# Vidvox/hap

Measured on AMD Instinct MI355X. Metric: RGBA GB/s + frames/sec, 8K Hap Q encode+decode, higher is better.
Workload: dtype u8; 1 GPU; C4: 7680x4320 0x1, 24 chunks, Snappy, 60-frame stream, device-resident; fragment_index=True, parallelism=single GPU

## Files before the change

hap_amd/csrc/bc_encode_core.hpp:

```cpp
#pragma once
#include <hip/hip_runtime.h>
#include <stdint.h>

#include "bc_refine_core.hpp"

namespace hapbc {

constexpr int kFmtDXT1 = 0, kFmtDXT5 = 1, kFmtYCoCg = 2, kFmtRGTC1 = 3;
constexpr int kFmtYCoCgAlpha = 4;

__device__ __forceinline__ int mad24(int a, int b, int c)
{
    int r;
    asm("v_mad_i32_i24 %0, %1, %2, %3" : "=v"(r) : "v"(a), "v"(b), "v"(c));
    return r;
}
template <int K>
__device__ __forceinline__ int mad24k(int a, int c)
{
    int r;
    asm("v_mad_i32_i24 %0, %1, %2, %3" : "=v"(r) : "v"(a), "i"(K), "v"(c));
    return r;
}

__device__ __forceinline__ int quant5(int v) { int t = mad24k<31>(v, 128); return (t + (t >> 8)) >> 8; }
__device__ __forceinline__ int quant6(int v) { int t = mad24k<63>(v, 128); return (t + (t >> 8)) >> 8; }
__device__ __forceinline__ int expand5(int q) { return (q << 3) | (q >> 2); }
__device__ __forceinline__ int expand6(int q) { return (q << 2) | (q >> 4); }

typedef unsigned short pk_u16 __attribute__((ext_vector_type(2)));
typedef short pk_i16 __attribute__((ext_vector_type(2)));

__device__ __forceinline__ pk_u16 pk_shl(pk_u16 v, unsigned sh)
{
    unsigned r;
    asm("v_pk_lshlrev_b16 %0, %1, %2 op_sel_hi:[0,1]" : "=v"(r) : "v"(sh), "v"(__builtin_bit_cast(unsigned, v)));
    return __builtin_bit_cast(pk_u16, r);
}


__device__ __forceinline__ unsigned ramp_codes(unsigned w)
{
    return w ^ (~((w >> 1) | (w >> 2)) & 0x249249u);
}

template <int BIAS = 0>
__device__ __forceinline__ uint2 alpha_block(const int (&a)[16])
{
    int lo = a[0], hi = a[0];
#pragma unroll
    for (int i = 1; i < 16; i++) {
        lo = min(lo, a[i]);
        hi = max(hi, a[i]);
    }
    const int a0 = hi, a1 = lo;
    unsigned lo24 = 0, hi24 = 0;
    if (a0 != a1) {
        const int d = a0 - a1;
        const unsigned m = (unsigned)(524288.0f * __builtin_amdgcn_rcpf((float)d)) + 1u;
        const int neg_m14 = -(int)(14u * m);
        const int start = mad24(a0, (int)(14u * m), (int)__umul24((unsigned)max(d - 6, 0), m)) + (1 << 20);
#pragma unroll
        for (int i = 0; i < 16; i++) {
            const unsigned r1 = (unsigned)mad24(a[i], neg_m14, start) >> 20;
            if (i < 8)
                lo24 = __builtin_amdgcn_alignbit(r1, lo24, 3);
            else
                hi24 = __builtin_amdgcn_alignbit(r1, hi24, 3);
        }
        lo24 = ramp_codes(lo24 >> 8);
        hi24 = ramp_codes(hi24 >> 8);
    }
    const unsigned long long bits = (unsigned long long)lo24 | ((unsigned long long)hi24 << 24);
    const unsigned long long v = (unsigned long long)(unsigned)(a0 + (a1 << 8) + BIAS * 257) | (bits << 16);
    return make_uint2((unsigned)v, (unsigned)(v >> 32));
}

struct projection {
    unsigned adir;
    unsigned flip;
    int start;
    int top;
    unsigned m24;
};

__device__ __forceinline__ unsigned index_scale(unsigned len2)
{
    unsigned m = (unsigned)(50331648.0f * __builtin_amdgcn_rcpf((float)len2));
    const int rem = (int)(50331648u - m * len2);
    m += (rem >= (int)len2 ? 1u : 0u) - (rem < 0 ? 1u : 0u);
    return m;
}

template <int CHANNELS = 3>
__device__ __forceinline__ projection make_projection(unsigned p0, unsigned p1)
{
    projection pr;
    int dir[CHANNELS];
    unsigned adir = 0, flip = 0;
    int neg = 0, base = 0;
#pragma unroll
    for (int c = 0; c < CHANNELS; c++) {
        const int a = (int)((p0 >> (8 * c)) & 255u), b = (int)((p1 >> (8 * c)) & 255u);
        dir[c] = a - b;
        const int ad = abs(dir[c]);
        adir |= (unsigned)ad << (8 * c);
        flip |= (dir[c] < 0 ? 0xFFu : 0u) << (8 * c);
        neg += dir[c] < 0 ? ad : 0;
        base = mad24(b, dir[c], base);
    }
    const unsigned len2 = __builtin_amdgcn_udot4(adir, adir, 0u, false);
    const unsigned sixth = __umulhi(len2, 0xAAAAAAABu) >> 2;
    pr.adir = adir;
    pr.flip = flip;
    pr.start = (int)sixth - base - 255 * neg;
    pr.top = (int)(len2 + sixth);
    pr.m24 = index_scale(len2);
    return pr;
}

#define HAPBC_CLAMPED_DOTS(OP)                                                                                           \
    asm(OP " %0, %4, %8, %9\n\t" OP " %1, %5, %8, %9\n\t" OP " %2, %6, %8, %9\n\t" OP " %3, %7, %8, %9\n\t"              \
        "v_med3_i32 %0, %0, 0, %10\n\tv_med3_i32 %1, %1, 0, %10\n\tv_med3_i32 %2, %2, 0, %10\n\tv_med3_i32 %3, %3, 0, %10" \
        : "=&v"(t[0]), "=&v"(t[1]), "=&v"(t[2]), "=&v"(t[3])                                                             \
        : "v"(q0), "v"(q1), "v"(q2), "v"(q3), "v"(dir), "v"(start), "v"(top))
__device__ __forceinline__ void clamped_dot4(unsigned (&t)[4], unsigned q0, unsigned q1, unsigned q2, unsigned q3, unsigned dir, int start, int top)
{
    HAPBC_CLAMPED_DOTS("v_dot4_u32_u8");
}
__device__ __forceinline__ void clamped_dot2(unsigned (&t)[4], unsigned q0, unsigned q1, unsigned q2, unsigned q3, unsigned dir, int start, int top)
{
    HAPBC_CLAMPED_DOTS("v_dot2_i32_i16");
}
#undef HAPBC_CLAMPED_DOTS

template <typename DOTS>
__device__ __forceinline__ unsigned gather_indices(unsigned m24, DOTS dots)
{
    const unsigned m30 = m24 << 6;
    unsigned pos2 = 0;
#pragma unroll
    for (int g = 3; g >= 0; g--) {
        unsigned t[4];
        dots(t, 4 * g);
#pragma unroll
        for (int k = 3; k >= 0; k--)
            pos2 = __builtin_amdgcn_alignbit(pos2, t[k] * m30, 30);
    }
    const unsigned hi = pos2 & 0xAAAAAAAAu;
    return (hi ^ ((pos2 << 1) & 0xAAAAAAAAu)) | ((~hi >> 1) & 0x55555555u);
}

template <bool FLIPPED = false>
__device__ __forceinline__ unsigned project4(const unsigned (&px)[16], const projection &pr)
{
    return gather_indices(pr.m24, [&](unsigned (&t)[4], int i) {
        clamped_dot4(t, FLIPPED ? px[i] : px[i] ^ pr.flip, FLIPPED ? px[i + 1] : px[i + 1] ^ pr.flip,
                     FLIPPED ? px[i + 2] : px[i + 2] ^ pr.flip, FLIPPED ? px[i + 3] : px[i + 3] ^ pr.flip, pr.adir, pr.start, pr.top);
    });
}

__device__ __forceinline__ unsigned pack3(int a, int b, int c) { return (unsigned)a | ((unsigned)b << 8) | ((unsigned)c << 16); }

__device__ __forceinline__ unsigned expand_565(unsigned c, bool blue)
{
    return pack3(expand5(c >> 11), expand6((c >> 5) & 63), blue ? expand5(c & 31) : 0);
}

template <bool REFINE = false>
__device__ __forceinline__ uint2 colour_block(const unsigned (&px)[16])
{
    int lo[3] = {255, 255, 255}, hi[3] = {0, 0, 0};
#pragma unroll
    for (int i = 0; i < 16; i++) {
#pragma unroll
        for (int c = 0; c < 3; c++) {
            const int v = (int)((px[i] >> (8 * c)) & 255u);
            lo[c] = min(lo[c], v);
            hi[c] = max(hi[c], v);
        }
    }
    int cov_rg = 0, cov_bg = 0;
    const int mr = lo[0] + hi[0], mg = lo[1] + hi[1], mb = lo[2] + hi[2];
#pragma unroll
    for (int i = 0; i < 16; i++) {
        const int dr = 2 * (int)(px[i] & 255u) - mr;
        const int dg = 2 * (int)((px[i] >> 8) & 255u) - mg;
        const int db = 2 * (int)((px[i] >> 16) & 255u) - mb;
        cov_rg = mad24(dr, dg, cov_rg);
        cov_bg = mad24(db, dg, cov_bg);
    }
#pragma unroll
    for (int c = 0; c < 3; c++) {
        const int inset = (hi[c] - lo[c]) >> 4;
        lo[c] += inset;
        hi[c] -= inset;
    }
    const int ar = cov_rg < 0 ? lo[0] : hi[0], br = cov_rg < 0 ? hi[0] : lo[0];
    const int ab = cov_bg < 0 ? lo[2] : hi[2], bb = cov_bg < 0 ? hi[2] : lo[2];
    const unsigned qa = (unsigned)(quant5(ar) << 11 | quant6(hi[1]) << 5 | quant5(ab));
    const unsigned qb = (unsigned)(quant5(br) << 11 | quant6(lo[1]) << 5 | quant5(bb));
    const unsigned c0 = max(qa, qb), c1 = min(qa, qb);
    unsigned idx = 0;
    if (c0 != c1)
        idx = project4(px, make_projection(expand_565(c0, true), expand_565(c1, true)));
    if constexpr (REFINE) {
        unsigned best0 = c0, best1 = c1, best_idx = idx;
        int best_rank = refine_rank(px, refine_make_palette(c0, c1), idx);
        const refine_sums plain = refine_plain_sums(px);
#pragma unroll
        for (int round = 0; round < 2; round++) {
            unsigned n0, n1, nidx = 0;
            const bool valid = refine_candidate(px, plain, refine_weights(best_idx), n0, n1);
            const refine_palette pal = refine_make_palette(n0, n1);
            if (valid && n0 != n1)
                nidx = project4(px, make_projection(pal.entry[0], pal.entry[1]));
            const int rank = refine_rank(px, pal, nidx);
            const bool win = valid && rank < best_rank;
            best0 = win ? n0 : best0;
            best1 = win ? n1 : best1;
            best_idx = win ? nidx : best_idx;
            best_rank = win ? rank : best_rank;
        }
        return make_uint2(best0 | (best1 << 16), best_idx);
    }
    return make_uint2(c0 | (c1 << 16), idx);
}

template <bool BIASED>
__device__ __forceinline__ uint2 ycocg_colour_block(const unsigned (&cc)[16])
{
    const auto pk_minimum3 = [](unsigned a, unsigned b, unsigned c) {
        unsigned r;
        asm("v_pk_minimum3_f16 %0, %1, %2, %3" : "=v"(r) : "v"(a), "v"(b), "v"(c));
        return r;
    };
    const auto pk_maximum3 = [](unsigned a, unsigned b, unsigned c) {
        unsigned r;
        asm("v_pk_maximum3_f16 %0, %1, %2, %3" : "=v"(r) : "v"(a), "v"(b), "v"(c));
        return r;
    };
    pk_i16 lo_b = __builtin_bit_cast(pk_i16, cc[0]), hi_b = lo_b;
    if (BIASED) {
        unsigned lo_w = pk_minimum3(cc[0], cc[1], cc[2]), hi_w = pk_maximum3(cc[0], cc[1], cc[2]);
#pragma unroll
        for (int i = 3; i < 15; i += 2) {
            lo_w = pk_minimum3(lo_w, cc[i], cc[i + 1]);
            hi_w = pk_maximum3(hi_w, cc[i], cc[i + 1]);
        }
        lo_b = __builtin_bit_cast(pk_i16, pk_minimum3(lo_w, cc[15], cc[15]));
        hi_b = __builtin_bit_cast(pk_i16, pk_maximum3(hi_w, cc[15], cc[15]));
    } else {
#pragma unroll
        for (int i = 1; i < 16; i++) {
            const pk_i16 v = __builtin_bit_cast(pk_i16, cc[i]);
            lo_b = __builtin_elementwise_min(lo_b, v);
            hi_b = __builtin_elementwise_max(hi_b, v);
        }
    }
    int prod = 0;
    unsigned sum_w = 0;
    pk_i16 sum_pk = {0, 0};
#pragma unroll
    for (int i = 0; i < 16; i++) {
        int r;
        asm("v_mad_i32_i16 %0, %1, %1, %2 op_sel:[0,1,0,0]" : "=v"(r) : "v"(cc[i]), "v"(prod));
        prod = r;
        if (BIASED)
            sum_w += cc[i];
        else
            sum_pk += __builtin_bit_cast(pk_i16, cc[i]);
    }
    const pk_i16 sums = BIASED ? __builtin_bit_cast(pk_i16, sum_w) : sum_pk;
    const pk_i16 mid = lo_b + hi_b;
    const pk_i16 rest = mid * (short)4 - sums;
    const int half_cov = __builtin_amdgcn_sdot2(rest, mid.yx, 2 * prod, false);
    const pk_i16 centre = {128, 128};
    const pk_i16 lo = BIASED ? lo_b - centre : lo_b, hi = BIASED ? hi_b - centre : hi_b;
    const pk_i16 mm = __builtin_elementwise_max((pk_i16)-lo, hi);
    const int m = max((int)mm.x, (int)mm.y);
    const unsigned sh = (unsigned)max(2 - (m >> 5), 0);
    const unsigned s1 = (1u << sh) - 1u;
    pk_u16 ls = pk_shl(__builtin_bit_cast(pk_u16, lo), sh), hs = pk_shl(__builtin_bit_cast(pk_u16, hi), sh);
    const pk_u16 ins = (pk_u16)(hs - ls) >> 4;
    ls += ins;
    hs -= ins;
    const unsigned cross = (unsigned)(half_cov >> 31) & 0xFFFF0000u, lsw = __builtin_bit_cast(unsigned, ls), hsw = __builtin_bit_cast(unsigned, hs);
    const pk_u16 end_a = __builtin_bit_cast(pk_u16, (lsw & cross) | (hsw & ~cross));
    const pk_u16 end_b = __builtin_bit_cast(pk_u16, (hsw & cross) | (lsw & ~cross));
    const pk_u16 q_mul = {31, 63}, q_add = {31 * 128 + 128, 63 * 128 + 128};
    const pk_u16 ta = end_a * q_mul + q_add, tb = end_b * q_mul + q_add;
    const pk_u16 pa = (pk_u16)(ta + (ta >> 8)) >> 8, pb = (pk_u16)(tb + (tb >> 8)) >> 8;
    const pk_u16 q_place = {1 << 11, 1 << 5};
    const unsigned qa = __builtin_amdgcn_udot2(pa, q_place, s1, false), qb = __builtin_amdgcn_udot2(pb, q_place, s1, false);
    const unsigned c0 = max(qa, qb), c1 = min(qa, qb);
    unsigned idx = 0;
    if (c0 != c1) {
        const bool sw = qa < qb;
        const pk_u16 q0 = sw ? pb : pa, q1 = sw ? pa : pb;
        const pk_u16 up = {3, 2}, down = {2, 4};
        const pk_u16 p0 = (q0 << up) | (q0 >> down), p1 = (q1 << up) | (q1 >> down);
        const pk_i16 dir = __builtin_bit_cast(pk_i16, (pk_u16)(p0 - p1)), back = __builtin_bit_cast(pk_i16, (pk_u16)(128 - p1));
        unsigned len2, dir2;
        int dot_back;
        if (BIASED)
            asm("v_dot2_i32_i16 %[len2], %[d], %[d], 0\n\tv_dot2_i32_i16 %[k], %[d], %[b], 0\n\t"
                "v_pk_lshlrev_b16 %[d2], %[sh], %[d] op_sel_hi:[0,1]\n\t"
                "v_dot2_i32_i16 %[k], %[d2], %[uncentre], %[k]\n\ts_nop 2"
                : [len2] "=&v"(len2), [k] "=&v"(dot_back), [d2] "=&v"(dir2)
                : [d] "v"(dir), [b] "v"(back), [sh] "v"(sh), [uncentre] "s"(0xFF80FF80u));
        else
            asm("v_dot2_i32_i16 %[len2], %[d], %[d], 0\n\tv_dot2_i32_i16 %[k], %[d], %[b], 0\n\t"
                "v_pk_lshlrev_b16 %[d2], %[sh], %[d] op_sel_hi:[0,1]\n\ts_nop 1"
                : [len2] "=&v"(len2), [k] "=&v"(dot_back), [d2] "=&v"(dir2)
                : [d] "v"(dir), [b] "v"(back), [sh] "v"(sh));
        const int sixth = (int)(__umulhi(len2, 0xAAAAAAABu) >> 2);
        const unsigned m24 = index_scale(len2);
        const int K = dot_back + sixth, top = (int)len2 + sixth;
        idx = gather_indices(m24, [&](unsigned (&t)[4], int i) { clamped_dot2(t, cc[i], cc[i + 1], cc[i + 2], cc[i + 3], dir2, K, top); });
    }
    return make_uint2(c0 | (c1 << 16), idx);
}

__device__ __forceinline__ uint2 ycocg_colour_block_scalar(const unsigned (&cc)[16])
{
    pk_i16 lo = __builtin_bit_cast(pk_i16, cc[0]), hi = lo;
#pragma unroll
    for (int i = 1; i < 16; i++) {
        const pk_i16 v = __builtin_bit_cast(pk_i16, cc[i]);
        lo = __builtin_elementwise_min(lo, v);
        hi = __builtin_elementwise_max(hi, v);
    }
    int lo_o = lo.x, hi_o = hi.x, lo_g = lo.y, hi_g = hi.y;
    const int m = max(max(-lo_o, hi_o), max(-lo_g, hi_g));
    const int s = m <= 31 ? 4 : (m <= 63 ? 2 : 1);
    int prod = 0;
    pk_i16 sums = {0, 0};
#pragma unroll
    for (int i = 0; i < 16; i++) {
        int r;
        asm("v_mad_i32_i16 %0, %1, %1, %2 op_sel:[0,1,0,0]" : "=v"(r) : "v"(cc[i]), "v"(prod));
        prod = r;
        sums += __builtin_bit_cast(pk_i16, cc[i]);
    }
    const int mo = lo_o + hi_o, mg = lo_g + hi_g;
    const int cov = 4 * prod - 2 * mg * (int)sums.x - 2 * mo * (int)sums.y + 16 * mo * mg;
    lo_o = lo_o * s + 128; hi_o = hi_o * s + 128;
    lo_g = lo_g * s + 128; hi_g = hi_g * s + 128;
    int ins = (hi_o - lo_o) >> 4; lo_o += ins; hi_o -= ins;
    ins = (hi_g - lo_g) >> 4; lo_g += ins; hi_g -= ins;
    const int ag = cov < 0 ? lo_g : hi_g, bg = cov < 0 ? hi_g : lo_g;
    const int qo_a = quant5(hi_o), qo_b = quant5(lo_o), qg_a = quant6(ag), qg_b = quant6(bg);
    const unsigned qa = (unsigned)(qo_a << 11 | qg_a << 5 | (s - 1));
    const unsigned qb = (unsigned)(qo_b << 11 | qg_b << 5 | (s - 1));
    const unsigned c0 = max(qa, qb), c1 = min(qa, qb);
    unsigned idx = 0;
    if (c0 != c1) {
        const bool sw = qa < qb;
        const int eo_a = expand5(qo_a), eo_b = expand5(qo_b), eg_a = expand6(qg_a), eg_b = expand6(qg_b);
        const int d_o = sw ? eo_b - eo_a : eo_a - eo_b, d_g = sw ? eg_b - eg_a : eg_a - eg_b;
        const int p1_o = sw ? eo_a : eo_b, p1_g = sw ? eg_a : eg_b;
        const unsigned len2 = (unsigned)mad24(d_o, d_o, __mul24(d_g, d_g));
        const int sixth = (int)(__umulhi(len2, 0xAAAAAAABu) >> 2);
        const unsigned m24 = index_scale(len2);
        const int K = mad24(d_o, 128 - p1_o, mad24(d_g, 128 - p1_g, sixth));
        const unsigned dir2 = ((unsigned)(d_o * s) & 0xFFFFu) | ((unsigned)(d_g * s) << 16);
        const int top = (int)len2 + sixth;
        idx = gather_indices(m24, [&](unsigned (&t)[4], int i) { clamped_dot2(t, cc[i], cc[i + 1], cc[i + 2], cc[i + 3], dir2, K, top); });
    }
    return make_uint2(c0 | (c1 << 16), idx);
}

typedef int mfma_i32x4 __attribute__((ext_vector_type(4)));

__device__ __forceinline__ unsigned ycocg_weight_rows()
{
    const unsigned row = threadIdx.x & 3u;
    const unsigned w = row == 0u ? 0x00010201u : (row == 1u ? 0x00FE0002u : (row == 2u ? 0x00FF02FFu : 0u));
    unsigned r;
    asm volatile("v_mov_b32 %0, %1" : "=v"(r) : "v"(w));
    return r;
}

__device__ __forceinline__ mfma_i32x4 ycocg_addend()
{
    mfma_i32x4 c = {2, 2 + 512, 2 + 512, 0};
    asm volatile("" : "+v"(c));
    return c;
}

#define HAPBC_YCOCG_MFMA "v_mfma_i32_4x4x4_16b_i8 "
#define HAPBC_YCOCG_SHIFT(CC) "v_pk_ashrrev_i16 " CC ", 2, " CC " op_sel_hi:[0,1]\n\t"
template <bool BIASED>
__device__ __forceinline__ void ycocg_pair_first(mfma_i32x4 &ta, mfma_i32x4 &tb, unsigned pa, unsigned pb, unsigned rows, const mfma_i32x4 &addend)
{
    unsigned qa, qb;
    if (BIASED)
        asm("v_xor_b32 %[qa], %[k80], %[pa]\n\tv_xor_b32 %[qb], %[k80], %[pb]\n\ts_nop 0\n\t"
            HAPBC_YCOCG_MFMA "%[ta], %[w], %[qa], %[c]\n\t" HAPBC_YCOCG_MFMA "%[tb], %[w], %[qb], %[c]\n\ts_nop 4"
            : [ta] "=&v"(ta), [tb] "=&v"(tb), [qa] "=&v"(qa), [qb] "=&v"(qb)
            : [pa] "v"(pa), [pb] "v"(pb), [w] "v"(rows), [c] "v"(addend), [k80] "s"(0x80808080u));
    else
        asm("v_xor_b32 %[qa], %[k80], %[pa]\n\tv_xor_b32 %[qb], %[k80], %[pb]\n\ts_nop 0\n\t"
            HAPBC_YCOCG_MFMA "%[ta], %[w], %[qa], 2\n\t" HAPBC_YCOCG_MFMA "%[tb], %[w], %[qb], 2\n\ts_nop 4"
            : [ta] "=&v"(ta), [tb] "=&v"(tb), [qa] "=&v"(qa), [qb] "=&v"(qb)
            : [pa] "v"(pa), [pb] "v"(pb), [w] "v"(rows), [k80] "s"(0x80808080u));
}
template <bool BIASED>
__device__ __forceinline__ void ycocg_pair(mfma_i32x4 &ta, mfma_i32x4 &tb, int &ya, int &yb, unsigned &cca, unsigned &ccb,
                                           unsigned pa, unsigned pb, unsigned rows, const mfma_i32x4 &addend)
{
    const mfma_i32x4 oa = ta, ob = tb;
    unsigned qa, qb;
    if (BIASED)
        asm("v_xor_b32 %[qa], %[k80], %[pa]\n\tv_xor_b32 %[qb], %[k80], %[pb]\n\t"
            "v_ashrrev_i32 %[ya], 2, %[oax]\n\tv_ashrrev_i32 %[yb], 2, %[obx]\n\t"
            "v_perm_b32 %[ca], %[oaz], %[oay], %[sel]\n\tv_perm_b32 %[cb], %[obz], %[oby], %[sel]\n\t"
            HAPBC_YCOCG_SHIFT("%[ca]")
            HAPBC_YCOCG_MFMA "%[ta], %[w], %[qa], %[c]\n\t" HAPBC_YCOCG_MFMA "%[tb], %[w], %[qb], %[c]\n\t"
            HAPBC_YCOCG_SHIFT("%[cb]") "s_nop 3"
            : [ta] "+v"(ta), [tb] "+v"(tb), [ya] "=&v"(ya), [yb] "=&v"(yb), [ca] "=&v"(cca), [cb] "=&v"(ccb), [qa] "=&v"(qa), [qb] "=&v"(qb)
            : [pa] "v"(pa), [pb] "v"(pb), [w] "v"(rows), [c] "v"(addend), [k80] "s"(0x80808080u), [sel] "s"(0x05040100),
              [oax] "v"(oa.x), [oay] "v"(oa.y), [oaz] "v"(oa.z), [obx] "v"(ob.x), [oby] "v"(ob.y), [obz] "v"(ob.z));
    else
        asm("v_xor_b32 %[qa], %[k80], %[pa]\n\tv_xor_b32 %[qb], %[k80], %[pb]\n\t"
            "v_ashrrev_i32 %[ya], 2, %[oax]\n\tv_ashrrev_i32 %[yb], 2, %[obx]\n\t"
            "v_perm_b32 %[ca], %[oaz], %[oay], %[sel]\n\tv_perm_b32 %[cb], %[obz], %[oby], %[sel]\n\t"
            HAPBC_YCOCG_SHIFT("%[ca]")
            HAPBC_YCOCG_MFMA "%[ta], %[w], %[qa], 2\n\t" HAPBC_YCOCG_MFMA "%[tb], %[w], %[qb], 2\n\t"
            HAPBC_YCOCG_SHIFT("%[cb]") "s_nop 3"
            : [ta] "+v"(ta), [tb] "+v"(tb), [ya] "=&v"(ya), [yb] "=&v"(yb), [ca] "=&v"(cca), [cb] "=&v"(ccb), [qa] "=&v"(qa), [qb] "=&v"(qb)
            : [pa] "v"(pa), [pb] "v"(pb), [w] "v"(rows), [k80] "s"(0x80808080u), [sel] "s"(0x05040100),
              [oax] "v"(oa.x), [oay] "v"(oa.y), [oaz] "v"(oa.z), [obx] "v"(ob.x), [oby] "v"(ob.y), [obz] "v"(ob.z));
}
__device__ __forceinline__ void ycocg_pair_last(int &ya, int &yb, unsigned &cca, unsigned &ccb, mfma_i32x4 oa, mfma_i32x4 ob)
{
    asm("v_ashrrev_i32 %[ya], 2, %[oax]\n\tv_ashrrev_i32 %[yb], 2, %[obx]\n\t"
        "v_perm_b32 %[ca], %[oaz], %[oay], %[sel]\n\tv_perm_b32 %[cb], %[obz], %[oby], %[sel]\n\t"
        HAPBC_YCOCG_SHIFT("%[ca]") "v_pk_ashrrev_i16 %[cb], 2, %[cb] op_sel_hi:[0,1]"
        : [ya] "=&v"(ya), [yb] "=&v"(yb), [ca] "=&v"(cca), [cb] "=&v"(ccb)
        : [sel] "s"(0x05040100), [oax] "v"(oa.x), [oay] "v"(oa.y), [oaz] "v"(oa.z), [obx] "v"(ob.x), [oby] "v"(ob.y), [obz] "v"(ob.z));
}
#undef HAPBC_YCOCG_SHIFT
#undef HAPBC_YCOCG_MFMA

__device__ __forceinline__ void chroma4(unsigned (&raw)[4], int q0, int q1, int q2, int q3)
{
    unsigned co[4];
    asm("v_dot4_i32_i8 %4, %8, %12, 1\n\tv_dot4_i32_i8 %0, %8, %13, 2\n\t"
        "v_dot4_i32_i8 %5, %9, %12, 1\n\tv_dot4_i32_i8 %1, %9, %13, 2\n\t"
        "v_dot4_i32_i8 %6, %10, %12, 1\n\tv_dot4_i32_i8 %2, %10, %13, 2\n\t"
        "v_dot4_i32_i8 %7, %11, %12, 1\n\tv_dot4_i32_i8 %3, %11, %13, 2\n\t"
        "v_perm_b32 %0, %0, %4, %14\n\tv_perm_b32 %1, %1, %5, %14\n\tv_perm_b32 %2, %2, %6, %14\n\tv_perm_b32 %3, %3, %7, %14"
        : "=&v"(raw[0]), "=&v"(raw[1]), "=&v"(raw[2]), "=&v"(raw[3]), "=&v"(co[0]), "=&v"(co[1]), "=&v"(co[2]), "=&v"(co[3])
        : "v"(q0), "v"(q1), "v"(q2), "v"(q3), "s"(0x00FF0001), "s"(0x00FF02FF), "s"(0x05040100));
}

template <int FMT, bool MATRIX = false, bool BIASED = false, bool REFINE = false>
__device__ __forceinline__ uint4 block_of(const unsigned (&p)[16], unsigned rows = 0u, const mfma_i32x4 &addend = mfma_i32x4{})
{
    static_assert(!REFINE || FMT == kFmtDXT1 || FMT == kFmtDXT5, "refined end points: the S3TC colour block only");
    if (FMT == kFmtRGTC1) {
        int a[16];
#pragma unroll
        for (int i = 0; i < 16; i++)
            a[i] = (int)(p[i] >> 24);
        const uint2 ab = alpha_block(a);
        return make_uint4(ab.x, ab.y, 0u, 0u);
    } else if (FMT == kFmtDXT1) {
        unsigned px[16];
#pragma unroll
        for (int i = 0; i < 16; i++)
            px[i] = p[i] & 0x00FFFFFFu;
        const uint2 cb = colour_block<REFINE>(px);
        return make_uint4(cb.x, cb.y, 0u, 0u);
    } else if (FMT == kFmtDXT5) {
        int a[16];
        unsigned px[16];
#pragma unroll
        for (int i = 0; i < 16; i++) {
            a[i] = (int)(p[i] >> 24);
            px[i] = p[i] & 0x00FFFFFFu;
        }
        const uint2 ab = alpha_block(a), cb = colour_block<REFINE>(px);
        return make_uint4(ab.x, ab.y, cb.x, cb.y);
    } else {
        int y[16];
        unsigned cc[16];
        if (MATRIX) {
            mfma_i32x4 ta, tb;
            ycocg_pair_first<BIASED>(ta, tb, p[0], p[1], rows, addend);
#pragma unroll
            for (int i = 2; i < 16; i += 2)
                ycocg_pair<BIASED>(ta, tb, y[i - 2], y[i - 1], cc[i - 2], cc[i - 1], p[i], p[i + 1], rows, addend);
            ycocg_pair_last(y[14], y[15], cc[14], cc[15], ta, tb);
        } else {
#pragma unroll
            for (int i = 0; i < 16; i++) {
                y[i] = (int)__builtin_amdgcn_udot4(p[i], 0x00010201u, (unsigned)(2 - 512), false) >> 2;
            }
#pragma unroll
            for (int i = 0; i < 16; i += 4) {
                unsigned raw[4];
                chroma4(raw, (int)(p[i] ^ 0x80808080u), (int)(p[i + 1] ^ 0x80808080u), (int)(p[i + 2] ^ 0x80808080u), (int)(p[i + 3] ^ 0x80808080u));
#pragma unroll
                for (int k = 0; k < 4; k++) {
                    const pk_i16 sh = {1, 2};
                    cc[i + k] = __builtin_bit_cast(unsigned, (pk_i16)(__builtin_bit_cast(pk_i16, raw[k]) >> sh));
                }
            }
        }
        const uint2 ab = alpha_block<128>(y), cb = MATRIX ? ycocg_colour_block<BIASED>(cc) : ycocg_colour_block_scalar(cc);
        return make_uint4(ab.x, ab.y, cb.x, cb.y);
    }
}

}
```

hap_amd/csrc/snappy_compress_blocks.hip:

```cpp
#include <hip/hip_runtime.h>
#include <stdint.h>
#include "hapgpu_runtime.hpp"
#include "measurement_guard.h"
#include "bc_encode_core.hpp"

namespace {

constexpr unsigned kFragBytes = 8192u;
constexpr unsigned kSteps = kFragBytes / 1024u;
constexpr unsigned kTableBits = 9u;
constexpr unsigned kDistances = 4u;

template <unsigned LAYOUT> struct unit_layout;
static_assert(HAPGPU_LAYOUT_2_6_4_4 == 4 && HAPGPU_LAYOUT_4_4 == 2 && HAPGPU_LAYOUT_2_6 == 6 && HAPGPU_LAYOUT_4_4_4_4 == 8,
              "the specialisations below are the layouts of hapgpu_abi.h");
static_assert(HAPGPU_FUSED_DXT1 == hapbc::kFmtDXT1 + 1 && HAPGPU_FUSED_DXT5 == hapbc::kFmtDXT5 + 1 &&
              HAPGPU_FUSED_YCOCG == hapbc::kFmtYCoCg + 1 && HAPGPU_FUSED_RGTC1 == hapbc::kFmtRGTC1 + 1 && HAPGPU_FUSED_NONE == 0,
              "snappy_compress_blocks_kernel compares the control word's kind with FUSED + 1");
template <> struct unit_layout<4u> {
    static constexpr unsigned block = 16u;
    static constexpr unsigned small32 = 0x11111111u;
    static constexpr unsigned big32 = 0x22222222u;
    static constexpr unsigned four32 = 0xCCCCCCCCu;
    static constexpr unsigned run3_12 = 0xBBBBBBBBu;
    static constexpr unsigned run15_61 = 0x22222222u;
    __device__ static constexpr unsigned fo(unsigned k) { return k == 0u ? 0u : k == 1u ? 2u : k == 2u ? 8u : 12u; }
    __device__ static constexpr unsigned fs(unsigned k) { return k == 0u ? 2u : k == 1u ? 6u : 4u; }
    __device__ static constexpr unsigned cls(unsigned k) { return k == 1u ? 1u : k == 3u ? 3u : 0u; }
    __device__ static unsigned pos(unsigned q) { const unsigned t = q << 1; return (t << 1) - (t & ~q & 2u); }
};
template <> struct unit_layout<2u> {
    static constexpr unsigned block = 8u;
    static constexpr unsigned small32 = 0u, big32 = 0u, four32 = 0xFFFFFFFFu, run3_12 = 0xFFFFFFFFu, run15_61 = 0u;
    __device__ static constexpr unsigned fo(unsigned k) { return 4u * k; }
    __device__ static constexpr unsigned fs(unsigned) { return 4u; }
    __device__ static constexpr unsigned cls(unsigned k) { return (k & 1u) ? 1u : 0u; }
    __device__ static unsigned pos(unsigned q) { return 4u * q; }
};
template <> struct unit_layout<8u> {
    static constexpr unsigned block = 16u;
    static constexpr unsigned small32 = 0u, big32 = 0u, four32 = 0xFFFFFFFFu, run3_12 = 0xFFFFFFFFu, run15_61 = 0u;
    __device__ static constexpr unsigned fo(unsigned k) { return 4u * k; }
    __device__ static constexpr unsigned fs(unsigned) { return 4u; }
    __device__ static constexpr unsigned cls(unsigned k) { return k == 1u ? 1u : k == 3u ? 3u : 0u; }
    __device__ static unsigned pos(unsigned q) { return 4u * q; }
};
template <> struct unit_layout<6u> {
    static constexpr unsigned block = 8u;
    static constexpr unsigned small32 = 0x55555555u, big32 = 0xAAAAAAAAu, four32 = 0u, run3_12 = 0xAAAAAAAAu,
                              run15_61 = 0xAAAAAAAAu;
    __device__ static constexpr unsigned fo(unsigned k) { return k == 0u ? 0u : k == 1u ? 2u : k == 2u ? 8u : 10u; }
    __device__ static constexpr unsigned fs(unsigned k) { return (k & 1u) ? 6u : 2u; }
    __device__ static constexpr unsigned cls(unsigned k) { return (k & 1u) ? 1u : 0u; }
    __device__ static unsigned pos(unsigned q) { return 4u * q - 2u * (q & 1u); }
};

typedef const uint8_t __attribute__((address_space(1))) *gsrc_t;
typedef uint8_t __attribute__((address_space(1))) *gdst_t;
struct __attribute__((packed)) pk_u16 { uint16_t v; };
struct __attribute__((packed)) pk_u32 { uint32_t v; };
struct __attribute__((packed)) pk_u64 { uint32_t a, b; };
struct __attribute__((packed)) pk_u128 { uint32_t a, b, c, d; };
__device__ __forceinline__ void put8(gdst_t p, unsigned v) { *p = (uint8_t)v; }
__device__ __forceinline__ void put16(gdst_t p, unsigned v) { reinterpret_cast<pk_u16 __attribute__((address_space(1))) *>(p)->v = (uint16_t)v; }
__device__ __forceinline__ void put32(gdst_t p, unsigned v) { reinterpret_cast<pk_u32 __attribute__((address_space(1))) *>(p)->v = v; }
__device__ __forceinline__ void put64(gdst_t p, uint2 v)
{
    pk_u64 __attribute__((address_space(1))) *q = reinterpret_cast<pk_u64 __attribute__((address_space(1))) *>(p);
    q->a = v.x; q->b = v.y;
}
__device__ __forceinline__ void put128(gdst_t p, uint4 v)
{
    pk_u128 __attribute__((address_space(1))) *q = reinterpret_cast<pk_u128 __attribute__((address_space(1))) *>(p);
    q->a = v.x; q->b = v.y; q->c = v.z; q->d = v.w;
}
__device__ __forceinline__ uint4 get128(gsrc_t p)
{
    const pk_u128 __attribute__((address_space(1))) *q = reinterpret_cast<const pk_u128 __attribute__((address_space(1))) *>(p);
    return make_uint4(q->a, q->b, q->c, q->d);
}
__device__ __forceinline__ uint2 get64(gsrc_t p)
{
    const pk_u64 __attribute__((address_space(1))) *q = reinterpret_cast<const pk_u64 __attribute__((address_space(1))) *>(p);
    return make_uint2(q->a, q->b);
}

__device__ __forceinline__ unsigned rotr(unsigned v, unsigned n) { return __builtin_amdgcn_alignbit(v, v, n); }
__device__ __forceinline__ unsigned bfi(unsigned mask, unsigned a, unsigned b) { return (a & mask) | (b & ~mask); }
__device__ __forceinline__ unsigned popc(unsigned v) { return (unsigned)__builtin_popcount(v); }
template <class UL>
__device__ __forceinline__ unsigned bytes_under(unsigned S, unsigned L, unsigned X3, unsigned under, unsigned base)
{
    const unsigned Lu = L & under;
    unsigned lit = popc(Lu) + popc(Lu & ~UL::small32);
    if (UL::big32 != 0u)
        lit += popc(Lu & UL::big32);
    return (base + popc(S & under) + popc(S & ~L & under) + popc(X3 & under)) + 2u * lit;
}
__device__ __forceinline__ unsigned bit_mask(unsigned v, unsigned bit) { return (unsigned)__builtin_amdgcn_sbfe((int)v, bit, 1u); }

__constant__ const unsigned kGroupInv[33] = {
    0u, 1048577u, 524289u, 349526u, 262145u, 209716u, 174763u, 149797u, 131073u, 116509u, 104858u,
    95326u, 87382u, 80660u, 74899u, 69906u, 65537u, 61681u, 58255u, 55189u, 52429u, 49933u,
    47663u, 45591u, 43691u, 41944u, 40330u, 38837u, 37450u, 36158u, 34953u, 33826u, 32769u};

__device__ __forceinline__ unsigned div_by(unsigned x, unsigned d, unsigned inv)
{
    const unsigned q = __umulhi(x, inv);
    return q + (x - q * d >= d ? 1u : 0u);
}

__device__ __forceinline__ int scan_add(int v)
{
    v += __builtin_amdgcn_update_dpp(0, v, 0x111, 0xF, 0xF, false);
    v += __builtin_amdgcn_update_dpp(0, v, 0x112, 0xF, 0xF, false);
    v += __builtin_amdgcn_update_dpp(0, v, 0x114, 0xF, 0xF, false);
    v += __builtin_amdgcn_update_dpp(0, v, 0x118, 0xF, 0xF, false);
    v += __builtin_amdgcn_update_dpp(0, v, 0x142, 0xA, 0xF, false);
    v += __builtin_amdgcn_update_dpp(0, v, 0x143, 0xC, 0xF, false);
    return v;
}

__device__ __forceinline__ unsigned lane_xor4(unsigned v)
{
    int t = __builtin_amdgcn_update_dpp(0, (int)v, 0x104, 0xF, 0x5, false);
    t = __builtin_amdgcn_update_dpp(t, (int)v, 0x114, 0xF, 0xA, false);
    return (unsigned)t;
}
__device__ __forceinline__ unsigned lane_xor2(unsigned v) { return (unsigned)__builtin_amdgcn_update_dpp(0, (int)v, 0x4E, 0xF, 0xF, false); }
__device__ __forceinline__ unsigned lane_xor1(unsigned v) { return (unsigned)__builtin_amdgcn_update_dpp(0, (int)v, 0xB1, 0xF, 0xF, false); }

typedef unsigned long long lanes_t;
__device__ __forceinline__ lanes_t ne32(unsigned a, unsigned b) { return __builtin_amdgcn_uicmp(a, b, 33); }
__device__ __forceinline__ lanes_t ne_lo16(unsigned a, unsigned b)
{
    lanes_t m;
    asm("v_cmp_ne_u32_sdwa %0, %1, %2 src0_sel:WORD_0 src1_sel:WORD_0" : "=s"(m) : "v"(a), "v"(b));
    return m;
}
__device__ __forceinline__ lanes_t ne_hi16(unsigned a, unsigned b)
{
    lanes_t m;
    asm("v_cmp_ne_u32_sdwa %0, %1, %2 src0_sel:WORD_1 src1_sel:WORD_1" : "=s"(m) : "v"(a), "v"(b));
    return m;
}
__device__ __forceinline__ unsigned shift_in(unsigned acc, lanes_t m)
{
    asm("v_addc_co_u32_e64 %0, %1, %0, %0, %1" : "+v"(acc), "+s"(m));
    return acc;
}

template <unsigned LAYOUT>
__device__ __forceinline__ unsigned differ_nibble(unsigned acc, const uint4 x, const uint4 y)
{
    lanes_t n0, n1, n2, n3;
    if (LAYOUT == 4u) {
        n0 = ne_lo16(x.x, y.x); n1 = ne_hi16(x.x, y.x) | ne32(x.y, y.y); n2 = ne32(x.z, y.z); n3 = ne32(x.w, y.w);
    } else if (LAYOUT == 2u || LAYOUT == 8u) {
        n0 = ne32(x.x, y.x); n1 = ne32(x.y, y.y); n2 = ne32(x.z, y.z); n3 = ne32(x.w, y.w);
    } else {
        n0 = ne_lo16(x.x, y.x); n1 = ne_hi16(x.x, y.x) | ne32(x.y, y.y);
        n2 = ne_lo16(x.z, y.z); n3 = ne_hi16(x.z, y.z) | ne32(x.w, y.w);
    }
    return shift_in(shift_in(shift_in(shift_in(acc, n3), n2), n1), n0);
}

template <unsigned LAYOUT>
__device__ __forceinline__ void index_field(const uint4 x, unsigned k, unsigned &lo, unsigned &hi)
{
    if (LAYOUT == 2u || LAYOUT == 8u) {
        lo = k == 1u ? x.y : x.w;
        hi = 0u;
    } else if (k == 1u) {
        lo = __builtin_amdgcn_alignbit(x.y, x.x, 16);
        hi = x.y >> 16;
    } else if (LAYOUT == 4u) {
        lo = x.w;
        hi = 0u;
    } else {
        lo = __builtin_amdgcn_alignbit(x.w, x.z, 16);
        hi = x.w >> 16;
    }
}

__device__ __forceinline__ unsigned table_slot(unsigned lo, unsigned hi, unsigned cls)
{
    const unsigned z = lo ^ rotr(hi, 19) ^ (cls << 29);
    return (z * 0x9E3779B1u) >> (32u - kTableBits);
}

#ifndef SCB_MIN_WAVES
#define SCB_MIN_WAVES 1
#endif
template <unsigned LAYOUT, int FUSED>
__global__ __launch_bounds__(64, (FUSED == hapbc::kFmtYCoCg && SCB_MIN_WAVES < 5) ? 5 : SCB_MIN_WAVES) void snappy_compress_blocks_kernel(const HapGpuFrameEnc *__restrict__ frames,
                                                                    uint8_t *__restrict__ slots, unsigned slot_stride,
                                                                    uint32_t *__restrict__ frag_sizes,
                                                                    uint8_t *__restrict__ group_tables, unsigned frames_inv)
{
    using UL = unit_layout<LAYOUT>;
    constexpr unsigned B = UL::block;
    __shared__ unsigned long long table[1u << kTableBits];
    __shared__ __attribute__((aligned(16))) uint32_t masks[64u * 8u];
    __shared__ uint32_t bounds[66];

    const unsigned lane = threadIdx.x;
    const unsigned ycocg_rows = FUSED == hapbc::kFmtYCoCg ? hapbc::ycocg_weight_rows() : 0u;
    const hapbc::mfma_i32x4 ycocg_add = FUSED == hapbc::kFmtYCoCg ? hapbc::ycocg_addend() : hapbc::mfma_i32x4{};
#ifdef PLC_NO_INTERLEAVE
    const unsigned zf = blockIdx.z, x = blockIdx.x;
#else
    const unsigned linear = blockIdx.z * gridDim.x + blockIdx.x;
    const unsigned round = div_by(linear, gridDim.z, frames_inv);
    const unsigned zf = gridDim.y == 1u ? linear - round * gridDim.z : blockIdx.z;
    const unsigned x = gridDim.y == 1u ? round : blockIdx.x;
#endif
    const HapGpuTexEnc tex = frames[zf].tex[blockIdx.y < 2u ? blockIdx.y : 0u];
    const unsigned tex_count = frames[zf].tex_count;
    if ((blockIdx.y >= tex_count) | (tex.compressor != 1u) | (hapgpu_control_layout(tex.control) != LAYOUT) |
        (x >= tex.chunk_count * tex.frags_per_chunk) | (tex.src == 0) | (tex.chunk_bytes == 0) |
        (hapgpu_control_fused(tex.control) != (unsigned)(FUSED + 1)))
        return;
    const unsigned chunk = div_by(x, tex.frags_per_chunk, tex.frags_per_chunk_inv), fj = x - chunk * tex.frags_per_chunk;
    const unsigned begin = fj * kFragBytes;
    const unsigned n = min(kFragBytes, tex.chunk_bytes - begin);
    const gsrc_t src = (gsrc_t)(tex.src + (uint64_t)chunk * tex.chunk_bytes + begin);
    const unsigned f = tex.frag_first + x;
    gdst_t out = (gdst_t)((uintptr_t)slots + (size_t)f * slot_stride);
    const bool placed = hapgpu_control_placed(tex.control) != 0u && blockIdx.y == 0u;
    const unsigned window = hapgpu_control_window_256(tex.control) ? hapgpu_control_window_256(tex.control) * 256u : 0xFFFFFFFFu;
    const bool want_sizes = hapgpu_control_half_tiles(tex.control) != 0u && group_tables != nullptr;
    gdst_t table_at = (gdst_t)((uintptr_t)group_tables + (size_t)f * HAP_GROUP_TABLE_BYTES);

    {
        uint4 *t = reinterpret_cast<uint4 *>(table);
#pragma unroll
        for (unsigned i = 0; i < (sizeof(table) / 16u) / 64u; i++)
            t[i * 64u + lane] = make_uint4(0, 0, 0, 0);
    }
    __syncthreads();

    const unsigned keep4 = (lane & 4u) ? 0xFFFF0000u : 0x0000FFFFu;
    const unsigned keep2 = (lane & 2u) ? 0xFF00FF00u : 0x00FF00FFu;
    const unsigned keep1 = (lane & 1u) ? 0xF0F0F0F0u : 0x0F0F0F0Fu;
    const unsigned rot2 = (lane & 2u) ? 8u : 24u;
    const unsigned rot1 = (lane & 1u) ? 4u : 28u;
    const unsigned last = n - (B == 16u ? 16u : 8u);

    constexpr unsigned kSub = 16u / B;
    __shared__ __attribute__((aligned(16))) uint4 ring[FUSED >= 0 ? 68u : 1u];
    const gsrc_t rgba = (gsrc_t)frames[zf].rgba;
    const unsigned row_bytes = frames[zf].rgba_row_bytes, blocks_x = frames[zf].rgba_blocks_x, blocks_x_inv = frames[zf].rgba_blocks_x_inv;
    unsigned bx[kSub], row_at[kSub], first_off = 0u;
#ifdef SCB_PREFETCH
    constexpr bool kPrefetch = SCB_PREFETCH != 0;
#else
    constexpr bool kPrefetch = FUSED != hapbc::kFmtYCoCg;
#endif
    unsigned pix[kPrefetch ? 2 : 1][16];
    auto whole_unit = [&](unsigned s) { return (int)lane < (int)(n >> 4) - (int)(64u * s); };
    unsigned long long row_base[4];
#pragma unroll
    for (unsigned r = 0; r < 4u; r++) {
        row_base[r] = (unsigned long long)(uintptr_t)rgba + (unsigned long long)r * row_bytes;
        asm("" : "+s"(row_base[r]));
    }
    auto load_pixels = [&](unsigned (&p)[16], unsigned t) {
        const unsigned sub = t % kSub;
        const bool there = B == 16u ? whole_unit(t) : (64u * t + lane + 1u) * B <= n;
        const unsigned at = there ? row_at[sub] + 16u * bx[sub] : first_off;
#pragma unroll
        for (unsigned r = 0; r < 4u; r++) {
            const uint4 v = get128((gsrc_t)(uintptr_t)row_base[r] + at);
            p[4u * r] = v.x; p[4u * r + 1u] = v.y; p[4u * r + 2u] = v.z; p[4u * r + 3u] = v.w;
        }
    };
    auto next_block = [&](unsigned sub) {
        bx[sub] += 64u * kSub;
        while (bx[sub] >= blocks_x) {
            bx[sub] -= blocks_x;
            row_at[sub] += 4u * row_bytes;
        }
    };
    if (FUSED >= 0) {
        const unsigned first_block = (unsigned)(((uint64_t)chunk * tex.chunk_bytes + begin) / B);
        {
            const unsigned fy = div_by(first_block, blocks_x, blocks_x_inv), fx = first_block - fy * blocks_x;
            first_off = (4u * fy) * row_bytes + 16u * fx;
        }
#pragma unroll
        for (unsigned j = 0; j < kSub; j++) {
            const unsigned b = first_block + 64u * j + lane;
            const unsigned by = div_by(b, blocks_x, blocks_x_inv);
            bx[j] = b - by * blocks_x;
            row_at[j] = (4u * by) * row_bytes;
        }
        load_pixels(pix[0], 0u);
    }

    constexpr bool kKeepX = !(FUSED >= 0 && B == 8u);
    uint4 X[kKeepX ? kSteps : 1u];
    unsigned HD[kSteps];
#pragma unroll
    for (unsigned s = 0; s < kSteps; s++) {
        const unsigned pos = (64u * s + lane) * 16u;
        if (kKeepX)
            X[s] = make_uint4(0, 0, 0, 0);
        HD[s] = 0u;
        if (64u * s * 16u >= n) {
            masks[64u * s + lane] = 0u;
            continue;
        }
        const unsigned pc = min(pos, last);
        uint4 xs, Y[kDistances];
        if (FUSED >= 0) {
            uint4 made = make_uint4(0, 0, 0, 0);
#pragma unroll
            for (unsigned sub = 0; sub < kSub; sub++) {
                const unsigned t = kSub * s + sub;
                if (!kPrefetch) {
                    if (t > 0u) {
                        if (t >= kSub)
                            next_block(t % kSub);
                        load_pixels(pix[0], t);
                    }
                } else if (t + 1u < kSub * kSteps && 64u * (t + 1u) * B < n) {
                    if (t + 1u >= kSub)
                        next_block((t + 1u) % kSub);
                    load_pixels(pix[(t + 1u) & 1u], t + 1u);
                }
                const uint4 blk = hapbc::block_of<FUSED, FUSED == hapbc::kFmtYCoCg, FUSED == hapbc::kFmtYCoCg>(pix[kPrefetch ? t & 1u : 0u], ycocg_rows, ycocg_add);
                made = blk;
                const unsigned bpos = (64u * t + lane) * B;
                if (B == 16u) {
                    if (bpos + 16u <= n && !placed)
                        put128((gdst_t)(uintptr_t)(src + bpos), blk);
                    ring[4u + lane] = blk;
                } else {
                    if (bpos + 8u <= n)
                        put64((gdst_t)(uintptr_t)(src + bpos), make_uint2(blk.x, blk.y));
                    reinterpret_cast<uint2 *>(ring)[8u + 64u * sub + lane] = make_uint2(blk.x, blk.y);
                }
            }
            __syncthreads();
            const uint8_t *rb = reinterpret_cast<const uint8_t *>(ring) + (4u + lane) * 16u;
            xs = B == 16u ? made : *reinterpret_cast<const uint4 *>(rb);
#pragma unroll
            for (unsigned d = 0; d < kDistances; d++) {
                if (B == 16u) {
                    Y[d] = *reinterpret_cast<const uint4 *>(rb - (d + 1u) * 16u);
                } else {
                    const uint2 ylo = *reinterpret_cast<const uint2 *>(rb - (d + 1u) * 8u), yhi = *reinterpret_cast<const uint2 *>(rb - (d + 1u) * 8u + 8u);
                    Y[d] = make_uint4(ylo.x, ylo.y, yhi.x, yhi.y);
                }
            }
            __syncthreads();
            if (lane >= 60u)
                ring[lane - 60u] = xs;
        } else if (B == 16u) {
            xs = get128(src + pc);
#pragma unroll
            for (unsigned d = 0; d < kDistances; d++) {
                const unsigned back = (d + 1u) * B;
                Y[d] = get128(src + (s == 0u ? max(pc, back) - back : pc - back));
            }
        } else {
            const uint2 lo = get64(src + pc), hi = get64(src + min(pos + 8u, last));
            xs = make_uint4(lo.x, lo.y, hi.x, hi.y);
#pragma unroll
            for (unsigned d = 0; d < kDistances; d++) {
                const unsigned back = (d + 1u) * B;
                if (s == 0u) {
                    const uint2 ylo = get64(src + max(pc, back) - back), yhi = get64(src + max(pc + 8u, back) - back);
                    Y[d] = make_uint4(ylo.x, ylo.y, yhi.x, yhi.y);
                } else {
                    Y[d] = get128(src + pc - back);
                }
            }
        }
        if (kKeepX)
            X[s] = xs;
        unsigned differ = 0;
#pragma unroll
        for (unsigned d = kDistances; d-- > 0u;)
            differ = differ_nibble<LAYOUT>(differ, xs, Y[d]);
        unsigned ok = (B == 16u ? whole_unit(s) : pos + 16u <= n) ? 0xFFFFu : 0u;
        if (B == 8u)
            ok = pos + 16u <= n ? 0xFFFFu : pos + 8u <= n ? 0x3333u : 0u;
        if (s == 0u) {
            if (B == 16u)
                ok &= (1u << (4u * min(lane, 4u))) - 1u;
            else
                ok &= lane == 0u ? 0x000Cu : lane == 1u ? 0x0CFFu : 0xFFFFu;
        }
        unsigned P = ~differ & ok;
        const unsigned eq_fixed = P;
        unsigned slot[2], klo[2], khi[2], valid[2];
        unsigned long long e[2];
#pragma unroll
        for (unsigned i = 0; i < 2u; i++) {
            const unsigned k = 2u * i + 1u;
            unsigned lo, hi;
            index_field<LAYOUT>(xs, k, lo, hi);
            klo[i] = lo;
            khi[i] = hi | (UL::cls(k) << 16);
            slot[i] = table_slot(lo, hi, UL::cls(k));
            valid[i] = (B == 16u ? whole_unit(s) : i == 0u ? pos + 8u <= n : pos + 16u <= n) ? 0xFFFFFFFFu : 0u;
            e[i] = table[slot[i]];
        }
        unsigned hd2[2];
#pragma unroll
        for (unsigned i = 0; i < 2u; i++) {
            const unsigned unit = 64u * s + lane;
            const unsigned blk = B == 16u ? unit : 2u * unit + i;
            const unsigned elo = (unsigned)e[i], ehi = (unsigned)(e[i] >> 32);
            const unsigned dist = blk - (ehi >> 18);
            const unsigned miss = (elo ^ klo[i]) | ((ehi & 0x3FFFFu) ^ khi[i]) | ~valid[i];
            const bool hit = (miss == 0u) & (dist * B <= window);
            hd2[i] = hit ? dist : 0u;
            P |= hit ? (dist * B >= 2048u ? 0x220000u : 0x020000u) << (2u * i) : 0u;
            const unsigned enter = valid[i] & ~(0u - ((eq_fixed >> (2u * i + 1u)) & 1u));
            atomicMax(&table[slot[i]], ((unsigned long long)((khi[i] | (blk << 18)) & enter) << 32) | (klo[i] & enter));
        }
        HD[s] = hd2[0] | (hd2[1] << 16);
        P = bfi(keep4, P, rotr(lane_xor4(P), 16));
        P = bfi(keep2, P, rotr(lane_xor2(P), rot2));
        P = bfi(keep1, P, rotr(lane_xor1(P), rot1));
        masks[64u * s + lane] = P;
    }
    __syncthreads();

    {
        uint32_t *hd_tab = reinterpret_cast<uint32_t *>(table);
#pragma unroll
        for (unsigned s = 0; s < kSteps; s++)
            hd_tab[64u * s + lane] = HD[s];
    }
    unsigned counts_and_bytes = 0;
    {
        const uint4 ma = *reinterpret_cast<const uint4 *>(&masks[lane * 8u]);
        const uint4 mb = *reinterpret_cast<const uint4 *>(&masks[lane * 8u + 4u]);
        const unsigned fields_total = (n >> 4) * 4u + ((n & 8u) ? 2u : 0u);
        const unsigned nv = fields_total > 32u * lane ? min(32u, fields_total - 32u * lane) : 0u;
        const unsigned valid = nv >= 32u ? 0xFFFFFFFFu : ((1u << nv) - 1u);
        unsigned E[kDistances] = {ma.x, ma.y, ma.z, ma.w}, A[kDistances] = {0u, 0u, 0u, 0u};
        unsigned U = 0;
#pragma unroll
        for (unsigned d = 0; d < kDistances; d++) {
            E[d] &= ~(UL::small32 & ~(E[d] >> 1) & ~(E[d] << 1));
            U |= E[d];
        }
        unsigned front = U & ~(U << 1);
        while (__builtin_amdgcn_ballot_w64(front != 0u) != 0ull) {
            unsigned taken = 0, ends = 0;
#pragma unroll
            for (unsigned dd = 0; dd < kDistances; dd++) {
#ifdef HAP_BLK_FAR_FIRST
                const unsigned d = kDistances - 1u - dd;
#else
                const unsigned d = dd;
#endif
                const unsigned seeds = front & E[d] & ~taken;
                const unsigned sum = E[d] + seeds;
                A[d] |= (E[d] & ~sum) | seeds;
                ends |= sum & ~E[d];
                taken |= seeds;
            }
            front = ends & U;
        }
        const unsigned cov = A[0] | A[1] | A[2] | A[3];
        unsigned Hm = mb.x & ~cov;
        unsigned L = valid & ~(cov | Hm);
        if (UL::four32 != 0u) {
            const unsigned cpy = cov | Hm;
            const unsigned lone4 = cpy & ~(cpy << 1) & ~(cpy >> 1) & UL::four32 & (L << 1) & (L >> 1);
            L |= lone4;
            Hm &= ~lone4;
#pragma unroll
            for (unsigned d = 0; d < kDistances; d++)
                A[d] &= ~lone4;
        }
        unsigned S = 0;
#pragma unroll
        for (int pass = 0; pass < 2; pass++) {
            S = Hm | (L & ~(L << 1));
#pragma unroll
            for (unsigned d = 0; d < kDistances; d++)
                S |= A[d] & ~(A[d] << 1);
            S &= valid;
            {
                const unsigned a = 31u - (unsigned)__builtin_clz((S & 0xFFFFu) | 1u);
                const unsigned b = 17u + (unsigned)__builtin_ctz(((S | ~valid) >> 17) | 0x8000u);
                const unsigned bytes = UL::pos(b) - UL::pos(a);
                const unsigned inside = (valid & ~S & ~L) >> 16;
                S |= (inside & (bytes > 64u ? 1u : 0u)) << 16;
            }
            if (pass == 0 && UL::small32 != 0u) {
                const unsigned lone = UL::small32 & S & (((S | ~valid) >> 1) | 0x80000000u) & ~L & ~Hm & valid;
                L |= lone;
#pragma unroll
                for (unsigned d = 0; d < kDistances; d++)
                    A[d] &= ~lone;
            }
        }
        const unsigned Sx1 = ((S | ~valid) >> 1) | 0x80000000u;
        const unsigned CS = S & ~L;
        const unsigned N1 = ~Sx1;
        const unsigned C3 = (CS & N1 & (N1 >> 1) & ((N1 >> 2) | UL::run3_12)) | (Hm & mb.y);
        const unsigned Cn = L & ~S;
        const unsigned w2 = Cn & (Cn >> 1), w4 = w2 & (w2 >> 2), w8 = w4 & (w4 >> 4);
// ... 242 lines not shown
```

Measured before the change: 2826 GB/s.

## Fold luma scaling into YCoCg MFMA weights and add negated-luma alpha block encoder

After: 2858 GB/s (median of 6 runs). +1.1%, better.

```diff
diff --git a/hap_amd/csrc/bc_encode_core.hpp b/hap_amd/csrc/bc_encode_core.hpp
--- a/hap_amd/csrc/bc_encode_core.hpp
+++ b/hap_amd/csrc/bc_encode_core.hpp
@@ -20,6 +20,19 @@
 {
     int r;
     asm("v_mad_i32_i24 %0, %1, %2, %3" : "=v"(r) : "v"(a), "i"(K), "v"(c));
+    return r;
+}
+__device__ __forceinline__ unsigned mad24u(unsigned a, unsigned b, unsigned c)
+{
+    unsigned r;
+    asm("v_mad_u32_u24 %0, %1, %2, %3" : "=v"(r) : "v"(a), "v"(b), "v"(c));
+    return r;
+}
+template <int K>
+__device__ __forceinline__ unsigned mad24uk(unsigned a)
+{
+    unsigned r;
+    asm("v_mad_u32_u24 %0, %1, %2, %2" : "=v"(r) : "v"(a), "i"(K));
     return r;
 }
 
@@ -74,6 +87,34 @@
     const unsigned long long bits = (unsigned long long)lo24 | ((unsigned long long)hi24 << 24);
     const unsigned long long v = (unsigned long long)(unsigned)(a0 + (a1 << 8) + BIAS * 257) | (bits << 16);
     return make_uint2((unsigned)v, (unsigned)(v >> 32));
+}
+
+__device__ __forceinline__ uint2 luma_block_negated(const unsigned (&v)[16])
+{
+    unsigned lo = v[0], hi = v[0];
+#pragma unroll
+    for (int i = 1; i < 16; i++) {
+        lo = min(lo, v[i]);
+        hi = max(hi, v[i]);
+    }
+    unsigned lo24 = 0, hi24 = 0;
+    if (lo != hi) {
+        const unsigned d = (hi - lo) >> 8;
+        const unsigned m1 = (unsigned)(524288.0f * __builtin_amdgcn_rcpf((float)d));
+        const unsigned m28 = mad24uk<28>(m1);
+        const unsigned d6 = (unsigned)max((int)d - 6, 0);
+        const unsigned start9 = ((mad24u(d6, m1, d6) << 9) + (1u << 29)) - mad24u(lo, m28, 0u);
+#pragma unroll
+        for (int i = 7; i >= 0; i--) {
+            lo24 = __builtin_amdgcn_alignbit(lo24, mad24u(v[i], m28, start9), 29);
+            hi24 = __builtin_amdgcn_alignbit(hi24, mad24u(v[i + 8], m28, start9), 29);
+        }
+        lo24 = ramp_codes(lo24);
+        hi24 = ramp_codes(hi24);
+    }
+    const unsigned long long bits = (unsigned long long)lo24 | ((unsigned long long)hi24 << 24);
+    const unsigned long long w = (unsigned long long)(((lo >> 8) | hi) ^ 0xFFFFu) | (bits << 16);
+    return make_uint2((unsigned)w, (unsigned)(w >> 32));
 }
 
 struct projection {
@@ -382,9 +423,18 @@
     return r;
 }
 
+__device__ __forceinline__ unsigned ycocg_weight_rows_biased()
+{
+    const unsigned row = threadIdx.x & 3u;
+    const unsigned w = row == 0u ? 0x00C080C0u : (row == 1u ? 0x00FE0002u : (row == 2u ? 0x00FF02FFu : 0u));
+    unsigned r;
+    asm volatile("v_mov_b32 %0, %1" : "=v"(r) : "v"(w));
+    return r;
+}
+
 __device__ __forceinline__ mfma_i32x4 ycocg_addend()
 {
-    mfma_i32x4 c = {2, 2 + 512, 2 + 512, 0};
+    mfma_i32x4 c = {32576, 2 + 512, 2 + 512, 0};
     asm volatile("" : "+v"(c));
     return c;
 }
@@ -414,13 +464,13 @@
     unsigned qa, qb;
     if (BIASED)
         asm("v_xor_b32 %[qa], %[k80], %[pa]\n\tv_xor_b32 %[qb], %[k80], %[pb]\n\t"
-            "v_ashrrev_i32 %[ya], 2, %[oax]\n\tv_ashrrev_i32 %[yb], 2, %[obx]\n\t"
+            "v_and_b32 %[ya], %[kff], %[oax]\n\tv_and_b32 %[yb], %[kff], %[obx]\n\t"
             "v_perm_b32 %[ca], %[oaz], %[oay], %[sel]\n\tv_perm_b32 %[cb], %[obz], %[oby], %[sel]\n\t"
             HAPBC_YCOCG_SHIFT("%[ca]")
             HAPBC_YCOCG_MFMA "%[ta], %[w], %[qa], %[c]\n\t" HAPBC_YCOCG_MFMA "%[tb], %[w], %[qb], %[c]\n\t"
             HAPBC_YCOCG_SHIFT("%[cb]") "s_nop 3"
             : [ta] "+v"(ta), [tb] "+v"(tb), [ya] "=&v"(ya), [yb] "=&v"(yb), [ca] "=&v"(cca), [cb] "=&v"(ccb), [qa] "=&v"(qa), [qb] "=&v"(qb)
-            : [pa] "v"(pa), [pb] "v"(pb), [w] "v"(rows), [c] "v"(addend), [k80] "s"(0x80808080u), [sel] "s"(0x05040100),
+            : [pa] "v"(pa), [pb] "v"(pb), [w] "v"(rows), [c] "v"(addend), [k80] "s"(0x80808080u), [kff] "s"(0xFF00u), [sel] "s"(0x05040100),
               [oax] "v"(oa.x), [oay] "v"(oa.y), [oaz] "v"(oa.z), [obx] "v"(ob.x), [oby] "v"(ob.y), [obz] "v"(ob.z));
     else
         asm("v_xor_b32 %[qa], %[k80], %[pa]\n\tv_xor_b32 %[qb], %[k80], %[pb]\n\t"
@@ -433,8 +483,16 @@
             : [pa] "v"(pa), [pb] "v"(pb), [w] "v"(rows), [k80] "s"(0x80808080u), [sel] "s"(0x05040100),
               [oax] "v"(oa.x), [oay] "v"(oa.y), [oaz] "v"(oa.z), [obx] "v"(ob.x), [oby] "v"(ob.y), [obz] "v"(ob.z));
 }
+template <bool BIASED>
 __device__ __forceinline__ void ycocg_pair_last(int &ya, int &yb, unsigned &cca, unsigned &ccb, mfma_i32x4 oa, mfma_i32x4 ob)
 {
+    if (BIASED)
+        asm("v_and_b32 %[ya], %[kff], %[oax]\n\tv_and_b32 %[yb], %[kff], %[obx]\n\t"
+            "v_perm_b32 %[ca], %[oaz], %[oay], %[sel]\n\tv_perm_b32 %[cb], %[obz], %[oby], %[sel]\n\t"
+            HAPBC_YCOCG_SHIFT("%[ca]") "v_pk_ashrrev_i16 %[cb], 2, %[cb] op_sel_hi:[0,1]"
+            : [ya] "=&v"(ya), [yb] "=&v"(yb), [ca] "=&v"(cca), [cb] "=&v"(ccb)
+            : [sel] "s"(0x05040100), [kff] "s"(0xFF00u), [oax] "v"(oa.x), [oay] "v"(oa.y), [oaz] "v"(oa.z), [obx] "v"(ob.x), [oby] "v"(ob.y), [obz] "v"(ob.z));
+    else
     asm("v_ashrrev_i32 %[ya], 2, %[oax]\n\tv_ashrrev_i32 %[yb], 2, %[obx]\n\t"
         "v_perm_b32 %[ca], %[oaz], %[oay], %[sel]\n\tv_perm_b32 %[cb], %[obz], %[oby], %[sel]\n\t"
         HAPBC_YCOCG_SHIFT("%[ca]") "v_pk_ashrrev_i16 %[cb], 2, %[cb] op_sel_hi:[0,1]"
@@ -493,7 +551,7 @@
 #pragma unroll
             for (int i = 2; i < 16; i += 2)
                 ycocg_pair<BIASED>(ta, tb, y[i - 2], y[i - 1], cc[i - 2], cc[i - 1], p[i], p[i + 1], rows, addend);
-            ycocg_pair_last(y[14], y[15], cc[14], cc[15], ta, tb);
+            ycocg_pair_last<BIASED>(y[14], y[15], cc[14], cc[15], ta, tb);
         } else {
 #pragma unroll
             for (int i = 0; i < 16; i++) {
@@ -510,7 +568,8 @@
                 }
             }
         }
-        const uint2 ab = alpha_block<128>(y), cb = MATRIX ? ycocg_colour_block<BIASED>(cc) : ycocg_colour_block_scalar(cc);
+        const uint2 ab = (MATRIX && BIASED) ? luma_block_negated(reinterpret_cast<const unsigned (&)[16]>(y)) : alpha_block<128>(y);
+        const uint2 cb = MATRIX ? ycocg_colour_block<BIASED>(cc) : ycocg_colour_block_scalar(cc);
         return make_uint4(ab.x, ab.y, cb.x, cb.y);
     }
 }
diff --git a/hap_amd/csrc/snappy_compress_blocks.hip b/hap_amd/csrc/snappy_compress_blocks.hip
--- a/hap_amd/csrc/snappy_compress_blocks.hip
+++ b/hap_amd/csrc/snappy_compress_blocks.hip
@@ -205,7 +205,7 @@
     __shared__ uint32_t bounds[66];
 
     const unsigned lane = threadIdx.x;
-    const unsigned ycocg_rows = FUSED == hapbc::kFmtYCoCg ? hapbc::ycocg_weight_rows() : 0u;
+    const unsigned ycocg_rows = FUSED == hapbc::kFmtYCoCg ? hapbc::ycocg_weight_rows_biased() : 0u;
     const hapbc::mfma_i32x4 ycocg_add = FUSED == hapbc::kFmtYCoCg ? hapbc::ycocg_addend() : hapbc::mfma_i32x4{};
 #ifdef PLC_NO_INTERLEAVE
     const unsigned zf = blockIdx.z, x = blockIdx.x;
```
